# GeWu-Lab/Crab

Hardware: AMD Instinct MI355X
Metric: clips/sec prefill+decode (AVQA 10s clip, 8 frames, 256 out tok) (higher is better)
Workload: dtype bf16

## Files before the change

crab_amd/csrc/attn.hip:

```cpp
#include "common.h"
#include "crab_internal.h"
#include "attn_decode_core.h"
#include <math.h>
#include <stdlib.h>

namespace {

struct AttnP {
    const bf16_t* q; const bf16_t* k; const bf16_t* vt; bf16_t* o;
    long q_bs, q_hs, q_ss, k_bs, k_hs, k_ss, vt_bs, vt_hs, vt_ds, o_bs, o_ss;
    const float* bias; const float* gate;
    const int* kv_start;
    const uint32_t* key_mask; long key_mask_ld;
    int B, H, Hk, Sq, Skv, causal;
    float scale;
};

constexpr int KT = 64;
constexpr int VT_LD = 68;

template <int HD>
__device__ __forceinline__ int k_swz(int row, int chunk) {
    return HD == 128 ? (chunk ^ (row & 15)) : (HD == 64 ? (chunk ^ ((row >> 1) & 7)) : (chunk ^ ((0x78 >> (((row >> 2) & 3) * 2)) & 3)));
}

template <int HD, bool CAUSAL, bool BIAS>
__global__ __launch_bounds__(256) void attn_fwd_kernel(AttnP p) {
    constexpr int CPR = HD / 8;
    constexpr int KS = HD / 32;
    constexpr int DT = HD / 16;
    __shared__ __attribute__((aligned(16))) bf16_t lk[KT * HD];
    __shared__ __attribute__((aligned(16))) bf16_t lv[HD * VT_LD];

    const int tid = threadIdx.x, lane = tid & 63, wave = tid >> 6;
    const int fr = lane & 15, fg = lane >> 4;
    const int nqb = (p.Sq + 63) >> 6;
    const int lid = xcd_remap(blockIdx.x, gridDim.x);
    const int b = lid / (nqb * p.H), h = (lid / nqb) % p.H;
    const int hk = h / (p.H / p.Hk);
    const int q0 = (lid % nqb) * 64;
    const int qrow = q0 + wave * 16 + fr;
    const int qload = qrow < p.Sq ? qrow : p.Sq - 1;
    const int koff = p.Skv - p.Sq;

    const bf16_t* qp = p.q + (long)b * p.q_bs + (long)h * p.q_hs + (long)qload * p.q_ss;
    const bf16_t* kp = p.k + (long)b * p.k_bs + (long)hk * p.k_hs;
    const bf16_t* vp = p.vt + (long)b * p.vt_bs + (long)hk * p.vt_hs;

    bf16x8_t qf[KS];
#pragma unroll
    for (int ks = 0; ks < KS; ++ks) qf[ks] = *reinterpret_cast<const bf16x8_t*>(qp + ks * 32 + fg * 8);

    f32x4_t oacc[DT];
#pragma unroll
    for (int i = 0; i < DT; ++i) oacc[i] = f32x4_t{0.f, 0.f, 0.f, 0.f};
    float m_run = -1e30f, l_run = 0.f;

    float gate = 1.f;
    const float* biasrow = nullptr;
    if (BIAS) {
        if (p.gate) gate = p.gate[((long)b * p.H + h) * p.Sq + qload];
        biasrow = p.bias + ((long)h * p.Sq + qload) * p.Skv;
    }

    int kv_end = p.Skv;
    if (CAUSAL) {
        int last = q0 + 63 + koff;
        if (last + 1 < kv_end) kv_end = last + 1;
    }
    const int ntiles = (kv_end + KT - 1) / KT;
    const int ks0 = p.kv_start ? p.kv_start[b] : 0;
    const int t0 = ks0 / KT;
    const uint32_t* km = p.key_mask ? p.key_mask + (long)b * p.key_mask_ld : nullptr;

    constexpr int NKV = (KT * CPR) / 256, NVV = (HD * 8) / 256;
    u32x4 kreg[NKV], vreg[NVV];
#define ATT_LOAD_TILE(T_)                                                                                      \
    {                                                                                                          \
        const int kvl_ = (T_) * KT;                                                                            \
        _Pragma("unroll") for (int i = 0; i < NKV; ++i) {                                                      \
            const int idx = tid + i * 256;                                                                     \
            const int row = idx / CPR, c = idx % CPR;                                                          \
            const int kr = min(kvl_ + row, p.Skv - 1);                                                         \
            kreg[i] = *reinterpret_cast<const u32x4*>(kp + (long)kr * p.k_ss + c * 8);                         \
        }                                                                                                      \
        _Pragma("unroll") for (int i = 0; i < NVV; ++i) {                                                      \
            const int idx = tid + i * 256;                                                                     \
            const int row = idx >> 3, c = idx & 7;                                                             \
            int kc = kvl_ + c * 8;                          \
            kc = kc < p.Skv ? kc : 0;                                                                          \
            vreg[i] = *reinterpret_cast<const u32x4*>(vp + (long)row * p.vt_ds + kc);                          \
        }                                                                                                      \
    }
#define ATT_MASK_V(T_)                                                                                         \
    if ((T_) * KT + KT > p.Skv) {                                                                              \
        _Pragma("unroll") for (int i = 0; i < NVV; ++i) {                                                      \
            const int c = (tid + i * 256) & 7;                                                                 \
            const int rem = p.Skv - ((T_) * KT + c * 8);         \
            _Pragma("unroll") for (int w = 0; w < 4; ++w) {                                                    \
                const uint32_t m = (2 * w < rem ? 0x0000ffffu : 0u) | (2 * w + 1 < rem ? 0xffff0000u : 0u);    \
                vreg[i][w] &= m;                                                                               \
            }                                                                                                  \
        }                                                                                                      \
    }
    if (t0 < ntiles) ATT_LOAD_TILE(t0)
    for (int t = t0; t < ntiles; ++t) {
        const int kv0 = t * KT;
        __syncthreads();
        ATT_MASK_V(t)
#pragma unroll
        for (int i = 0; i < NKV; ++i) {
            const int idx = tid + i * 256;
            const int row = idx / CPR, c = idx % CPR;
            *reinterpret_cast<u32x4*>(lk + row * HD + (k_swz<HD>(row, c) << 3)) = kreg[i];
        }
#pragma unroll
        for (int i = 0; i < NVV; ++i) {
            const int idx = tid + i * 256;
            const int row = idx >> 3, c = idx & 7;
            bf16_t* d = lv + row * VT_LD + c * 8;
            *reinterpret_cast<u32x2*>(d) = u32x2{vreg[i][0], vreg[i][1]};
            *reinterpret_cast<u32x2*>(d + 4) = u32x2{vreg[i][2], vreg[i][3]};
        }
        __syncthreads();
        if (t + 1 < ntiles) ATT_LOAD_TILE(t + 1);

        f32x4_t s[4];
#pragma unroll
        for (int j = 0; j < 4; ++j) {
            s[j] = f32x4_t{0.f, 0.f, 0.f, 0.f};
#pragma unroll
            for (int ks = 0; ks < KS; ++ks) {
                int row = j * 16 + fr;
                int chunk = ks * 4 + fg;
                bf16x8_t kf = *reinterpret_cast<const bf16x8_t*>(lk + row * HD + (k_swz<HD>(row, chunk) << 3));
                s[j] = __builtin_amdgcn_mfma_f32_16x16x32_bf16(kf, qf[ks], s[j], 0, 0, 0);
            }
        }
        const float sc2 = p.scale * 1.4426950408889634f;
        const bool need_mask = (kv0 + KT > p.Skv) || (CAUSAL && (kv0 + KT - 1 > q0 + wave * 16 + koff)) || (kv0 < ks0) || km;
        float tmax = -1e30f;
        if (BIAS || need_mask) {
#pragma unroll
            for (int j = 0; j < 4; ++j) {
#pragma unroll
                for (int r = 0; r < 4; ++r) {
                    int kv = kv0 + j * 16 + fg * 4 + r;
                    float v = s[j][r] * sc2;
                    if (BIAS) { if (kv < p.Skv) v += gate * biasrow[kv] * 1.4426950408889634f; }
                    bool ok = kv < p.Skv && kv >= ks0;
// ... 14 lines not shown
        tmax = fmaxf(tmax, __shfl_xor(tmax, 16, 64));
        tmax = fmaxf(tmax, __shfl_xor(tmax, 32, 64));
        const float m_new = fmaxf(m_run, tmax);
        const float alpha = __builtin_amdgcn_exp2f(m_run - m_new);
        m_run = m_new;
        float psum = 0.f;
#pragma unroll
        for (int j = 0; j < 4; ++j)
#pragma unroll
            for (int r = 0; r < 4; ++r) {
                float e = __builtin_amdgcn_exp2f(s[j][r] - m_new);
                s[j][r] = e;
                psum += e;
            }
        l_run = l_run * alpha + psum;
#pragma unroll
        for (int i = 0; i < DT; ++i) oacc[i] *= alpha;

#pragma unroll
        for (int kk = 0; kk < 2; ++kk) {
            union { bf16x8_t v; uint32_t w[4]; } pf;
            pf.w[0] = pack_bf2(s[2 * kk][0], s[2 * kk][1]);
            pf.w[1] = pack_bf2(s[2 * kk][2], s[2 * kk][3]);
            pf.w[2] = pack_bf2(s[2 * kk + 1][0], s[2 * kk + 1][1]);
            pf.w[3] = pack_bf2(s[2 * kk + 1][2], s[2 * kk + 1][3]);
#pragma unroll
            for (int dt = 0; dt < DT; ++dt) {
                const bf16_t* vr = lv + (dt * 16 + fr) * VT_LD + kk * 32 + fg * 4;
                union { bf16x8_t v; u32x2 h[2]; } vf;
                vf.h[0] = *reinterpret_cast<const u32x2*>(vr);
                vf.h[1] = *reinterpret_cast<const u32x2*>(vr + 16);
                oacc[dt] = __builtin_amdgcn_mfma_f32_16x16x32_bf16(vf.v, pf.v, oacc[dt], 0, 0, 0);
            }
        }
    }
    l_run += __shfl_xor(l_run, 16, 64);
    l_run += __shfl_xor(l_run, 32, 64);
    const float inv = l_run > 0.f ? 1.0f / l_run : 0.f;
    if (qrow < p.Sq) {
        bf16_t* op = p.o + (long)b * p.o_bs + (long)qrow * p.o_ss + (long)h * HD;
#pragma unroll
        for (int dt = 0; dt < DT; ++dt) {
            u32x2 w;
            w[0] = pack_bf2(oacc[dt][0] * inv, oacc[dt][1] * inv);
            w[1] = pack_bf2(oacc[dt][2] * inv, oacc[dt][3] * inv);
            *reinterpret_cast<u32x2*>(op + dt * 16 + fg * 4) = w;
        }
    }
}


typedef __attribute__((ext_vector_type(16))) float f32x16_t;

template <int HD, bool CAUSAL>
__global__ __launch_bounds__(256, 2) void attn_fwd32_kernel(AttnP p) {
    constexpr int CPR = HD / 8;
    constexpr int KS = HD / 16;
    constexpr int DT = HD / 32;
    constexpr int KBUF = KT * HD, VBUF = HD * VT_LD;
    __shared__ __attribute__((aligned(16))) bf16_t lk[2 * KBUF];
    __shared__ __attribute__((aligned(16))) bf16_t lv[2 * VBUF];

    const int tid = threadIdx.x, lane = tid & 63;
    const int wave = __builtin_amdgcn_readfirstlane(tid >> 6);
    const int fc = lane & 31, fg = lane >> 5;
    const int nqb = (p.Sq + 127) >> 7;
    const int lid = xcd_remap(blockIdx.x, gridDim.x);
    const int b = lid / (nqb * p.H), h = (lid / nqb) % p.H;
    const int hk = h / (p.H / p.Hk);
    const int q0 = (nqb - 1 - lid % nqb) * 128;
    const int qw0 = q0 + wave * 32;
    const int qrow = qw0 + fc;
    const int qload = qrow < p.Sq ? qrow : p.Sq - 1;
    const int koff = p.Skv - p.Sq;
    const bool wave_on = qw0 < p.Sq;

    const bf16_t* qp = p.q + (long)b * p.q_bs + (long)h * p.q_hs + (long)qload * p.q_ss;
    const bf16_t* kp = p.k + (long)b * p.k_bs + (long)hk * p.k_hs;
    const bf16_t* vp = p.vt + (long)b * p.vt_bs + (long)hk * p.vt_hs;

    bf16x8_t qf[KS];
#pragma unroll
    for (int ks = 0; ks < KS; ++ks) qf[ks] = *reinterpret_cast<const bf16x8_t*>(qp + ks * 16 + fg * 8);

    f32x16_t oacc[DT];
#pragma unroll
    for (int i = 0; i < DT; ++i)
#pragma unroll
        for (int r = 0; r < 16; ++r) oacc[i][r] = 0.f;
    float m_run = -1e30f, l_run = 0.f;

    int kv_end = p.Skv;
    if (CAUSAL) kv_end = min(kv_end, q0 + 128 + koff);
    const int ntiles = (kv_end + KT - 1) / KT;
    const int ks0 = p.kv_start ? p.kv_start[b] : 0;
    const int t0 = ks0 / KT;
    const uint32_t* km = p.key_mask ? p.key_mask + (long)b * p.key_mask_ld : nullptr;
    constexpr int NKV = (KT * CPR) / 256, NVV = (HD * 8) / 256;
    u32x4 kreg[NKV], vreg[NVV];
#define ATT_STORE_TILE(BUF_, T_)                                                                               \
    {                                                                                                          \
        ATT_MASK_V(T_)                                                                                         \
        bf16_t* lk_ = lk + (BUF_) * KBUF;                                                                      \
        bf16_t* lv_ = lv + (BUF_) * VBUF;                                                                      \
        _Pragma("unroll") for (int i = 0; i < NKV; ++i) {                                                      \
            const int idx = tid + i * 256;                                                                     \
            const int row = idx / CPR, c = idx % CPR;                                                          \
            *reinterpret_cast<u32x4*>(lk_ + row * HD + (k_swz<HD>(row, c) << 3)) = kreg[i];                    \
        }                                                                                                      \
        _Pragma("unroll") for (int i = 0; i < NVV; ++i) {                                                      \
            const int idx = tid + i * 256;                                                                     \
            const int row = idx >> 3, c = idx & 7;                                                             \
            bf16_t* d_ = lv_ + row * VT_LD + c * 8;                                                            \
            *reinterpret_cast<u32x2*>(d_) = u32x2{vreg[i][0], vreg[i][1]};                                     \
            *reinterpret_cast<u32x2*>(d_ + 4) = u32x2{vreg[i][2], vreg[i][3]};                                 \
        }                                                                                                      \
    }
    if (t0 >= ntiles) {
        if (qrow < p.Sq) {
            bf16_t* op = p.o + (long)b * p.o_bs + (long)qrow * p.o_ss + (long)h * HD;
#pragma unroll
            for (int c = 0; c < HD / 4; ++c) *reinterpret_cast<u32x2*>(op + c * 4 + 0) = u32x2{0u, 0u};
        }
        return;
    }
    ATT_LOAD_TILE(t0)
    ATT_STORE_TILE(0, t0)
    if (t0 + 1 < ntiles) ATT_LOAD_TILE(t0 + 1)
    __syncthreads();
    const float sc2 = p.scale * 1.4426950408889634f;
    for (int t = t0; t < ntiles; ++t) {
        const int cur = (t - t0) & 1;
        const int kv0 = t * KT;
        if (t + 1 < ntiles) {
            ATT_STORE_TILE(cur ^ 1, t + 1)
            if (t + 2 < ntiles) ATT_LOAD_TILE(t + 2)
        }
        const bool skip = !wave_on || (CAUSAL && kv0 > qw0 + 31 + koff);
        if (!skip) {
            const bf16_t* lkc = lk + cur * KBUF;
            const bf16_t* lvc = lv + cur * VBUF;
            f32x16_t s[2];
#pragma unroll
            for (int j = 0; j < 2; ++j)
#pragma unroll
                for (int r = 0; r < 16; ++r) s[j][r] = 0.f;
#pragma unroll
            for (int ks = 0; ks < KS; ++ks) {
#pragma unroll
                for (int j = 0; j < 2; ++j) {
                    const int row = j * 32 + fc;
                    const int chunk = ks * 2 + fg;
                    bf16x8_t kf = *reinterpret_cast<const bf16x8_t*>(lkc + row * HD + (k_swz<HD>(row, chunk) << 3));
                    s[j] = __builtin_amdgcn_mfma_f32_32x32x16_bf16(kf, qf[ks], s[j], 0, 0, 0);
                }
            }
            const bool need_mask = (kv0 + KT > p.Skv) || (CAUSAL && (kv0 + KT - 1 > qw0 + koff)) || (kv0 < ks0) || km;
            if (need_mask) {
#pragma unroll
                for (int j = 0; j < 2; ++j)
#pragma unroll
                    for (int r = 0; r < 16; ++r) {
                        const int kv = kv0 + j * 32 + (r >> 2) * 8 + fg * 4 + (r & 3);
                        bool ok = kv < p.Skv && kv >= ks0;
                        if (CAUSAL) ok = ok && (kv <= qrow + koff);
                        if (km) ok = ok && ((km[min(kv, p.Skv - 1) >> 5] >> (kv & 31)) & 1u);
                        s[j][r] = ok ? s[j][r] : -INFINITY;
                    }
            }
            float tmax = -INFINITY;
#pragma unroll
            for (int j = 0; j < 2; ++j)
#pragma unroll
                for (int r = 0; r < 16; r += 2) tmax = fmaxf(tmax, fmaxf(s[j][r], s[j][r + 1]));
            tmax = fmaxf(tmax, __shfl_xor(tmax, 32, 64));
            const float m_new = fmaxf(m_run, tmax * sc2);
            const float alpha = __builtin_amdgcn_exp2f(m_run - m_new);
            const bool raised = m_new != m_run;
            m_run = m_new;
            float psum = 0.f;
#pragma unroll
            for (int j = 0; j < 2; ++j)
#pragma unroll
                for (int r = 0; r < 16; ++r) {
                    const float e = __builtin_amdgcn_exp2f(__builtin_fmaf(s[j][r], sc2, -m_new));
                    s[j][r] = e;
                    psum += e;
                }
            l_run = l_run * alpha + psum;
            if (__any(raised)) {
#pragma unroll
                for (int i = 0; i < DT; ++i) oacc[i] *= alpha;
            }
#pragma unroll
            for (int j = 0; j < 2; ++j)
#pragma unroll
                for (int kk = 0; kk < 2; ++kk) {
                    union { bf16x8_t v; uint32_t w[4]; } pf;
                    pf.w[0] = pack_bf2(s[j][8 * kk + 0], s[j][8 * kk + 1]);
                    pf.w[1] = pack_bf2(s[j][8 * kk + 2], s[j][8 * kk + 3]);
                    pf.w[2] = pack_bf2(s[j][8 * kk + 4], s[j][8 * kk + 5]);
                    pf.w[3] = pack_bf2(s[j][8 * kk + 6], s[j][8 * kk + 7]);
#pragma unroll
                    for (int dt = 0; dt < DT; ++dt) {
                        const bf16_t* vr = lvc + (dt * 32 + fc) * VT_LD + j * 32 + kk * 16 + fg * 4;
                        union { bf16x8_t v; u32x2 hh[2]; } vf;
                        vf.hh[0] = *reinterpret_cast<const u32x2*>(vr);
                        vf.hh[1] = *reinterpret_cast<const u32x2*>(vr + 8);
                        oacc[dt] = __builtin_amdgcn_mfma_f32_32x32x16_bf16(vf.v, pf.v, oacc[dt], 0, 0, 0);
                    }
                }
        }
        __syncthreads();
    }
    l_run += __shfl_xor(l_run, 32, 64);
    const float inv = l_run > 0.f ? 1.0f / l_run : 0.f;
    if (qrow < p.Sq) {
        bf16_t* op = p.o + (long)b * p.o_bs + (long)qrow * p.o_ss + (long)h * HD;
#pragma unroll
        for (int dt = 0; dt < DT; ++dt)
#pragma unroll
            for (int g4 = 0; g4 < 4; ++g4) {
                u32x2 w;
                w[0] = pack_bf2(oacc[dt][4 * g4 + 0] * inv, oacc[dt][4 * g4 + 1] * inv);
                w[1] = pack_bf2(oacc[dt][4 * g4 + 2] * inv, oacc[dt][4 * g4 + 3] * inv);
                *reinterpret_cast<u32x2*>(op + dt * 32 + g4 * 8 + fg * 4) = w;
            }
    }
}
#undef ATT_LOAD_TILE
#undef ATT_MASK_V
#undef ATT_STORE_TILE

template <int HD>
__global__ __launch_bounds__(256) void attn_decode_kernel(const bf16_t* __restrict__ q, long ldq, const bf16_t* __restrict__ kc,
                                                          const bf16_t* __restrict__ vc, bf16_t* __restrict__ o, long ldo, int H, int Hk,
                                                          int Tmax, int ctx_host, const int* __restrict__ ctx_dev, float scale,
                                                          const int* __restrict__ kv_start) {
    constexpr int EPL = HD / 16;
    const int tid = threadIdx.x;
    const int grp = tid >> 4, sub = tid & 15;
    const int b = blockIdx.y, h = blockIdx.x;
    const int hk = h / (H / Hk);
    const int ks0 = kv_start ? kv_start[b] : 0;
    const int ctx = ctx_host + (ctx_dev ? ctx_dev[0] : 0) - ks0;
    const bf16_t* qp = q + (long)b * ldq + (long)h * HD + sub * EPL;
    float qv[EPL];
#pragma unroll
    for (int e = 0; e < EPL; ++e) qv[e] = bf2f(qp[e]) * scale;
    const bf16_t* kb = kc + (((long)b * Hk + hk) * (long)Tmax + ks0) * HD + sub * EPL;
    const bf16_t* vb = vc + (((long)b * Hk + hk) * (long)Tmax + ks0) * HD + sub * EPL;
    float m = -1e30f, l = 0.f, acc[EPL];
#pragma unroll
    for (int e = 0; e < EPL; ++e) acc[e] = 0.f;
    if constexpr (EPL == 8) {
        dec_stream(qv, kb, vb, ctx, grp, m, l, acc);
    } else {
        for (int j = grp; j < ctx; j += 16) {
            float kx[EPL], vx[EPL];
            const u32x2 kw = __builtin_nontemporal_load(reinterpret_cast<const u32x2*>(kb + (long)j * HD));
            const u32x2 vw = __builtin_nontemporal_load(reinterpret_cast<const u32x2*>(vb + (long)j * HD));
#pragma unroll
            for (int e = 0; e < 2; ++e) { kx[2 * e] = lo_bf(kw[e]); kx[2 * e + 1] = hi_bf(kw[e]); vx[2 * e] = lo_bf(vw[e]); vx[2 * e + 1] = hi_bf(vw[e]); }
            float sdot = 0.f;
#pragma unroll
            for (int e = 0; e < EPL; ++e) sdot += qv[e] * kx[e];
            sdot = row16_sum(sdot);
            const float mn = fmaxf(m, sdot);
            const float a = __expf(m - mn), pw = __expf(sdot - mn);
            l = l * a + pw;
#pragma unroll
            for (int e = 0; e < EPL; ++e) acc[e] = acc[e] * a + pw * vx[e];
            m = mn;
        }
    }
    float M, L, O;
    dec_group_merge<HD, 16, EPL>(grp, sub, m, l, acc, M, L, O);
    if (tid < HD) o[(long)b * ldo + (long)h * HD + tid] = f2bf(O / L);
}


template <int HD>
__global__ __launch_bounds__(256) void attn_decode_keymask_kernel(const bf16_t* __restrict__ q, long ldq, const bf16_t* __restrict__ kc,
                                                                  const bf16_t* __restrict__ vc, bf16_t* __restrict__ o, long ldo, int H, int Hk,
                                                                  int Tmax, int ctx_host, const int* __restrict__ ctx_dev, float scale,
// ... 344 lines not shown
        }
        for (int r0 = 0; r0 < rounds; r0 += RPT) {
            if (r0 > 0) {
#pragma unroll
                for (int u = 0; u < RPT; ++u) {
                    const int jc = min((r0 + u) * 16 + grp, cn - 1);
                    vw[u] = __builtin_nontemporal_load(reinterpret_cast<const u32x4*>(vb + (long)(c0 + jc) * HD));
                }
            }
#pragma unroll
            for (int u = 0; u < RPT; ++u) {
                const int j = (r0 + u) * 16 + grp, jc = min(j, cn - 1);
                f32x4_t p0 = *reinterpret_cast<const f32x4_t*>(sbuf + jc * 8);
                f32x4_t p1 = *reinterpret_cast<const f32x4_t*>(sbuf + jc * 8 + 4);
                if (j >= cn) { p0 = f32x4_t{0.f, 0.f, 0.f, 0.f}; p1 = f32x4_t{0.f, 0.f, 0.f, 0.f}; }
                float vx[EPL];
#pragma unroll
                for (int e = 0; e < 4; ++e) { vx[2 * e] = lo_bf(vw[u][e]); vx[2 * e + 1] = hi_bf(vw[u][e]); }
#pragma unroll
                for (int g = 0; g < G; ++g) {
                    const float pg = g < 4 ? p0[g & 3] : p1[g & 3];
#pragma unroll
                    for (int e = 0; e < EPL; ++e) acc[g][e] += pg * vx[e];
                }
            }
        }
    }
    __syncthreads();
#pragma unroll
    for (int g = 0; g < G; ++g)
#pragma unroll
        for (int e = 0; e < EPL; ++e) {
            float v = acc[g][e];
            v += __shfl_xor(v, 16, 64);
            v += __shfl_xor(v, 32, 64);
            acc[g][e] = v;
        }
    if (lane < 16) {
#pragma unroll
        for (int g = 0; g < G; ++g)
#pragma unroll
            for (int e = 0; e < EPL; ++e) sbuf[(wave * G + g) * HD + sub * EPL + e] = acc[g][e];
    }
    __syncthreads();
    for (int idx = tid; idx < G * HD; idx += 256) {
        const float O = (sbuf[idx] + sbuf[G * HD + idx]) + (sbuf[2 * G * HD + idx] + sbuf[3 * G * HD + idx]);
        const int g = idx / HD;
        o[(long)b * ldo + (long)(hk * G) * HD + idx] = f2bf(O / l_run[g]);
    }
}

}

extern "C" int crab_attn_fwd(crab_ctx* ctx, void* stream, const crab_attn_desc* d) {
    if (!ctx) return CRAB_E_INVALID;
    if (!d || !d->q || !d->k || !d->vt || !d->o) return crab_fail(ctx, CRAB_E_INVALID, "attn_fwd: null operand");
    if (d->B <= 0 || d->H <= 0 || d->Hk <= 0 || d->H % d->Hk || d->Sq <= 0 || d->Skv <= 0)
        return crab_fail(ctx, CRAB_E_INVALID, "attn_fwd: bad shape");
    if (d->head_dim != 32 && d->head_dim != 64 && d->head_dim != 128) return crab_fail(ctx, CRAB_E_UNSUPPORTED, "attn_fwd: head_dim must be 32, 64 or 128");
    if (d->head_dim == 32 && (d->causal || d->bias)) return crab_fail(ctx, CRAB_E_UNSUPPORTED, "attn_fwd: head_dim 32 only without mask/bias");
    if ((d->q_ss & 7) || (d->q_hs & 7) || (d->q_bs & 7) || (d->k_ss & 7) || (d->k_hs & 7) || (d->k_bs & 7) || (d->vt_ds & 7) ||
        (d->vt_hs & 7) || (d->vt_bs & 7) || (d->o_ss & 3) || (d->o_bs & 3))
        return crab_fail(ctx, CRAB_E_INVALID, "attn_fwd: strides must keep 16-byte alignment");
    if (((uintptr_t)d->q & 15) || ((uintptr_t)d->k & 15) || ((uintptr_t)d->vt & 15) || ((uintptr_t)d->o & 7))
        return crab_fail(ctx, CRAB_E_INVALID, "attn_fwd: pointer alignment");
    if (d->causal && d->Skv < d->Sq) return crab_fail(ctx, CRAB_E_INVALID, "attn_fwd: causal needs Skv >= Sq");
    if ((d->bias == nullptr) && d->gate) return crab_fail(ctx, CRAB_E_INVALID, "attn_fwd: gate without bias");
    if (d->key_mask && (d->key_mask_ld < (d->Skv + 31) / 32 || d->head_dim == 32))
        return crab_fail(ctx, CRAB_E_INVALID, "attn_fwd: key_mask needs key_mask_ld >= ceil(Skv / 32) words per sequence (head_dim 64 / 128)");
    AttnP p;
    p.q = (const bf16_t*)d->q; p.k = (const bf16_t*)d->k; p.vt = (const bf16_t*)d->vt; p.o = (bf16_t*)d->o;
    p.q_bs = d->q_bs; p.q_hs = d->q_hs; p.q_ss = d->q_ss; p.k_bs = d->k_bs; p.k_hs = d->k_hs; p.k_ss = d->k_ss;
    p.vt_bs = d->vt_bs; p.vt_hs = d->vt_hs; p.vt_ds = d->vt_ds; p.o_bs = d->o_bs; p.o_ss = d->o_ss;
    p.bias = d->bias; p.gate = d->gate; p.kv_start = d->kv_start; p.key_mask = d->key_mask; p.key_mask_ld = d->key_mask_ld; p.B = d->B; p.H = d->H; p.Hk = d->Hk; p.Sq = d->Sq; p.Skv = d->Skv;
    p.causal = d->causal; p.scale = d->scale;
    dim3 grid(((d->Sq + 63) / 64) * d->H * d->B), block(256);
    hipStream_t s = (hipStream_t)stream;
    const bool hb = d->bias != nullptr;
    if (d->causal && hb) return crab_fail(ctx, CRAB_E_UNSUPPORTED, "attn_fwd: causal + bias not instantiated");
    static const int fwd32 = []() { const char* e = getenv("CRAB_ATTN_FWD32"); return !(e && e[0] == '0'); }();
    if (fwd32 && !hb && d->Sq > 64 && d->scale > 0.f && (d->head_dim == 128 || d->head_dim == 64)) {
        dim3 grid32(((d->Sq + 127) / 128) * d->H * d->B);
        if (d->head_dim == 128) {
            if (d->causal) hipLaunchKernelGGL((attn_fwd32_kernel<128, true>), grid32, block, 0, s, p);
            else hipLaunchKernelGGL((attn_fwd32_kernel<128, false>), grid32, block, 0, s, p);
        } else {
            if (d->causal) hipLaunchKernelGGL((attn_fwd32_kernel<64, true>), grid32, block, 0, s, p);
            else hipLaunchKernelGGL((attn_fwd32_kernel<64, false>), grid32, block, 0, s, p);
        }
        return crab_check_launch(ctx, d->head_dim == 128 ? (d->causal ? "attn_fwd32_kernel<128,causal>" : "attn_fwd32_kernel<128>")
                                                         : (d->causal ? "attn_fwd32_kernel<64,causal>" : "attn_fwd32_kernel<64>"));
    }
    if (d->head_dim == 32) {
        hipLaunchKernelGGL((attn_fwd_kernel<32, false, false>), grid, block, 0, s, p);
    } else if (d->head_dim == 128) {
        if (d->causal) hipLaunchKernelGGL((attn_fwd_kernel<128, true, false>), grid, block, 0, s, p);
        else if (hb) hipLaunchKernelGGL((attn_fwd_kernel<128, false, true>), grid, block, 0, s, p);
        else hipLaunchKernelGGL((attn_fwd_kernel<128, false, false>), grid, block, 0, s, p);
    } else {
        if (d->causal) hipLaunchKernelGGL((attn_fwd_kernel<64, true, false>), grid, block, 0, s, p);
        else if (hb) hipLaunchKernelGGL((attn_fwd_kernel<64, false, true>), grid, block, 0, s, p);
        else hipLaunchKernelGGL((attn_fwd_kernel<64, false, false>), grid, block, 0, s, p);
    }
    return crab_check_launch(ctx, d->head_dim == 32 ? "attn_fwd_kernel<32>" : d->head_dim == 128 ? (d->causal ? "attn_fwd_kernel<128,causal>" : hb ? "attn_fwd_kernel<128,bias>" : "attn_fwd_kernel<128>")
                                                                            : (d->causal ? "attn_fwd_kernel<64,causal>" : hb ? "attn_fwd_kernel<64,bias>" : "attn_fwd_kernel<64>"));
}

extern "C" int64_t crab_attn_decode_rope_workspace(int B, int H, int d) {
    return ((int64_t)B * H * 8 * (d + 2) * 4 + 255) / 256 * 256 + (int64_t)B * H * 4;
}

extern "C" int crab_attn_decode_rope(crab_ctx* ctx, void* stream, const void* qkv, int64_t ldqkv, const float* rope_tab, void* k_cache,
                                     void* v_cache, void* o, int64_t ldo, int B, int H, int Hk, int d, int Tmax, int pos0,
                                     const int32_t* pos_dev, float scale, void* workspace, int64_t workspace_bytes) {
    if (!ctx) return CRAB_E_INVALID;
    if (!qkv || !rope_tab || !k_cache || !v_cache || !o || B <= 0 || H <= 0 || Hk <= 0 || H % Hk) return crab_fail(ctx, CRAB_E_INVALID, "attn_decode_rope: bad argument");
    if (d != 64 && d != 128) return crab_fail(ctx, CRAB_E_UNSUPPORTED, "attn_decode_rope: head_dim must be 64 or 128");
    if ((ldqkv & 7) || ((uintptr_t)qkv & 15) || ((uintptr_t)k_cache & 15) || ((uintptr_t)v_cache & 15)) return crab_fail(ctx, CRAB_E_INVALID, "attn_decode_rope: alignment");
    if (!pos_dev && (pos0 < 0 || pos0 >= Tmax)) return crab_fail(ctx, CRAB_E_INVALID, "attn_decode_rope: position outside the KV cache");
    int nsplit = 1;
    static const int tgt = []() { const char* e = getenv("CRAB_ATTN_BLOCKS"); return e ? atoi(e) : 512; }();
    if ((long)B * H < tgt) { nsplit = (int)(tgt / ((long)B * H)); if (nsplit > 8) nsplit = 8; }
    if (nsplit > 1 && (!workspace || workspace_bytes < crab_attn_decode_rope_workspace(B, H, d)))
        return crab_fail(ctx, CRAB_E_WORKSPACE, "attn_decode_rope: needs crab_attn_decode_rope_workspace(B, H, d) bytes (counters zeroed once)");
    float* part = (float*)workspace;
    unsigned* counters = workspace ? (unsigned*)((char*)workspace + ((int64_t)B * H * 8 * (d + 2) * 4 + 255) / 256 * 256) : nullptr;
    hipStream_t s = (hipStream_t)stream;
    static const int wide_on = []() { const char* e = getenv("CRAB_ATTN_WIDE"); return !(e && e[0] == '0'); }();
    if (wide_on && nsplit == 2 && d == 128) {
        hipLaunchKernelGGL((attn_decode_rope_kernel<128, 32>), dim3(H, B, 1), dim3(512), 0, s, (const bf16_t*)qkv, (long)ldqkv, rope_tab, (bf16_t*)k_cache,
                           (bf16_t*)v_cache, (bf16_t*)o, (long)ldo, H, Hk, Tmax, pos0, pos_dev, scale, (float*)nullptr, (unsigned*)nullptr);
        return crab_check_launch(ctx, "attn_decode_rope_kernel<128,32>");
    }
    dim3 grid(H, B, nsplit), block(256);
    if (d == 128)
        hipLaunchKernelGGL((attn_decode_rope_kernel<128>), grid, block, 0, s, (const bf16_t*)qkv, (long)ldqkv, rope_tab, (bf16_t*)k_cache,
                           (bf16_t*)v_cache, (bf16_t*)o, (long)ldo, H, Hk, Tmax, pos0, pos_dev, scale, part, counters);
    else
        hipLaunchKernelGGL((attn_decode_rope_kernel<64>), grid, block, 0, s, (const bf16_t*)qkv, (long)ldqkv, rope_tab, (bf16_t*)k_cache,
                           (bf16_t*)v_cache, (bf16_t*)o, (long)ldo, H, Hk, Tmax, pos0, pos_dev, scale, part, counters);
    return crab_check_launch(ctx, d == 128 ? "attn_decode_rope_kernel<128>" : "attn_decode_rope_kernel<64>");
}

extern "C" int crab_attn_decode_keymask(crab_ctx* ctx, void* stream, const void* q, int64_t ldq, const void* k_cache, const void* v_cache,
                                        void* o, int64_t ldo, int B, int H, int Hk, int d, int Tmax, int ctx_len_host, const int32_t* ctx_dev,
                                        float scale, const uint32_t* key_mask, int64_t key_mask_ld) {
    if (!ctx) return CRAB_E_INVALID;
    if (!q || !k_cache || !v_cache || !o || !key_mask || B <= 0 || H <= 0 || Hk <= 0 || H % Hk) return crab_fail(ctx, CRAB_E_INVALID, "attn_decode_keymask: bad argument");
    if (d != 64 && d != 128) return crab_fail(ctx, CRAB_E_UNSUPPORTED, "attn_decode_keymask: head_dim must be 64 or 128");
    if (!ctx_dev && (ctx_len_host <= 0 || ctx_len_host > Tmax)) return crab_fail(ctx, CRAB_E_INVALID, "attn_decode_keymask: ctx_len out of range");
    if (key_mask_ld < ((ctx_dev ? Tmax : ctx_len_host) + 31) / 32)
        return crab_fail(ctx, CRAB_E_INVALID, "attn_decode_keymask: key_mask_ld must cover the visible context (ceil(ctx_len / 32) words, Tmax with ctx_dev)");
    dim3 grid(H, B), block(256);
    hipStream_t s = (hipStream_t)stream;
    if (d == 128)
        hipLaunchKernelGGL((attn_decode_keymask_kernel<128>), grid, block, 0, s, (const bf16_t*)q, (long)ldq, (const bf16_t*)k_cache, (const bf16_t*)v_cache,
                           (bf16_t*)o, (long)ldo, H, Hk, Tmax, ctx_len_host, ctx_dev, scale, key_mask, (long)key_mask_ld);
    else
        hipLaunchKernelGGL((attn_decode_keymask_kernel<64>), grid, block, 0, s, (const bf16_t*)q, (long)ldq, (const bf16_t*)k_cache, (const bf16_t*)v_cache,
// ... 38 lines not shown
```

crab_amd/csrc/crab_internal.h:

```cpp
#pragma once
#include <hip/hip_runtime.h>
#include <stdio.h>
#include <string.h>
#include "../../include/crab_hip.h"

#define CRAB_TRACE_MAX 160
struct crab_trace_row { char name[64]; long count; };
struct crab_ctx {
    int device;
    char err[512];
    int trace_on;
    int trace_n;
    crab_trace_row trace[CRAB_TRACE_MAX];
};

static inline void crab_trace_note(crab_ctx* ctx, const char* what) {
    for (int i = 0; i < ctx->trace_n; ++i)
        if (strncmp(ctx->trace[i].name, what, sizeof(ctx->trace[i].name) - 1) == 0) { ++ctx->trace[i].count; return; }
    if (ctx->trace_n >= CRAB_TRACE_MAX) return;
    crab_trace_row* r = &ctx->trace[ctx->trace_n++];
    strncpy(r->name, what, sizeof(r->name) - 1);
    r->name[sizeof(r->name) - 1] = 0;
    r->count = 1;
}

static inline int crab_fail(crab_ctx* ctx, int code, const char* msg) {
    if (ctx) { strncpy(ctx->err, msg, sizeof(ctx->err) - 1); ctx->err[sizeof(ctx->err) - 1] = 0; }
    return code;
}

static inline int crab_check_launch(crab_ctx* ctx, const char* what) {
    hipError_t e = hipGetLastError();
    if (e != hipSuccess) {
        if (ctx) snprintf(ctx->err, sizeof(ctx->err), "%s: %s", what, hipGetErrorString(e));
        return CRAB_E_HIP;
    }
    if (ctx && ctx->trace_on) crab_trace_note(ctx, what);
    return CRAB_OK;
}

#define CRAB_HIP_TRY(ctx, expr)                                                                  \
    do {                                                                                         \
        hipError_t _e = (expr);                                                                  \
        if (_e != hipSuccess) {                                                                  \
            if (ctx) snprintf((ctx)->err, sizeof((ctx)->err), "%s: %s", #expr, hipGetErrorString(_e)); \
            return CRAB_E_HIP;                                                                   \
        }                                                                                        \
    } while (0)

static inline int crab_cflags(const crab_gemm_desc* d) { return (d->c_fp32 ? 1 : 0) | ((d->r_fp32 && d->R) ? 2 : 0); }

bool crab_rowfin_enabled();
extern "C" int crab_rowfin_lora_ok(int nl, int r, int N);
```

crab_amd/csrc/encoder_layers.hip:

```cpp
#include "crab_internal.h"
#include <math.h>

namespace {

int dense(crab_ctx* ctx, void* stream, const crab_enc_io* io, const crab_dense* w, const void* a, int64_t lda, void* c, int64_t ldc, int M, int act,
          const void* residual, int64_t ldr, float res_scale, int c_fp32 = 0, int r_fp32 = 0) {
    crab_gemm_desc d;
    memset(&d, 0, sizeof(d));
    d.A = a; d.lda = lda; d.B = w->W; d.ldb = w->ldw; d.C = c; d.ldc = ldc; d.bias = w->bias;
    d.R = residual; d.ldr = ldr; d.res_scale = res_scale; d.c_fp32 = c_fp32; d.r_fp32 = residual ? r_fp32 : 0;
    d.M = M; d.N = w->N; d.K = w->K; d.act = act; d.batch = 1; d.nb0 = 1;
    if (M <= CRAB_DECODE_MAX_ROWS) { d.workspace = io->workspace; d.workspace_bytes = io->workspace_bytes; }
    return crab_gemm_bf16(ctx, stream, &d);
}

int attention(crab_ctx* ctx, void* stream, const crab_enc_io* io, const uint16_t* q, int64_t ldq, const uint16_t* k, int64_t ldk,
              void* vsrc, int64_t ldv, int v_skip, int B, int H, int Sq, int Skv, int d, const float* bias, const float* gate) {
    const int Sp = (Skv + 7) / 8 * 8;
    if ((int64_t)B * H * d * Sp * 2 > io->vt_bytes) return crab_fail(ctx, CRAB_E_WORKSPACE, "encoder layer: vt scratch smaller than B * H * d * round8(Skv) * 2 bytes");
    int rc = crab_qkv_rope_split(ctx, stream, vsrc, ldv, nullptr, nullptr, nullptr, io->vt, Sp, B, Skv, v_skip, H, d, 1, 0, nullptr);
    if (rc) return rc;
    crab_attn_desc a;
    memset(&a, 0, sizeof(a));
    a.q = q; a.k = k; a.vt = io->vt; a.o = io->att;
    a.q_bs = (int64_t)Sq * ldq; a.q_hs = d; a.q_ss = ldq;
    a.k_bs = (int64_t)Skv * ldk; a.k_hs = d; a.k_ss = ldk;
    a.vt_bs = (int64_t)H * d * Sp; a.vt_hs = (int64_t)d * Sp; a.vt_ds = Sp;
    a.o_bs = (int64_t)Sq * H * d; a.o_ss = (int64_t)H * d;
    a.bias = bias; a.gate = gate;
    a.B = B; a.H = H; a.Hk = H; a.Sq = Sq; a.Skv = Skv; a.head_dim = d; a.causal = 0;
    a.scale = (float)(1.0 / sqrt((double)d));
    return crab_attn_fwd(ctx, stream, &a);
}

int ln(crab_ctx* ctx, void* stream, int x_fp32, const void* x, int64_t ldx, const crab_ln* w, void* y, int64_t ldy, int M, int D) {
    return crab_layernorm_p(ctx, stream, x, x_fp32, ldx, w->w, w->b, w->fp32, y, ldy, M, D, w->eps);
}

int check_io(crab_ctx* ctx, const crab_enc_io* io, bool need_f, const char* who) {
    char msg[160];
    if (!io || !io->x || !io->a || !io->qkv || !io->att || !io->vt || !io->y || (need_f && !io->f) || io->B <= 0 || io->S <= 0) {
        snprintf(msg, sizeof(msg), "%s: x, a, qkv, att, vt, y%s and positive B, S are required", who, need_f ? ", f" : "");
        return crab_fail(ctx, CRAB_E_INVALID, msg);
    }
    return CRAB_OK;
}

}

extern "C" {

int crab_clip_layer(crab_ctx* ctx, void* stream, const crab_clip_layer_w* w, crab_enc_io* io) {
    if (!ctx) return CRAB_E_INVALID;
    if (!w) return crab_fail(ctx, CRAB_E_INVALID, "clip_layer: null weights");
    int rc = check_io(ctx, io, true, "clip_layer");
    if (rc) return rc;
    const int D = w->out.N, H = w->H, M = io->B * io->S;
    if (H <= 0 || D % H || w->qkv.N != 3 * D || w->qkv.K != D || w->out.K != D || w->fc1.K != D || w->fc2.N != D || w->fc2.K != w->fc1.N)
        return crab_fail(ctx, CRAB_E_INVALID, "clip_layer: shapes do not chain (qkv [3D, D], out [D, D], fc1 [I, D], fc2 [D, I])");
    const int d = D / H;
    uint16_t* qkv = (uint16_t*)io->qkv;
    const int xf = io->x_fp32 ? 1 : 0;
    if ((rc = ln(ctx, stream, xf, io->x, D, &w->ln1, io->a, D, M, D))) return rc;
    if ((rc = dense(ctx, stream, io, &w->qkv, io->a, D, qkv, 3 * D, M, CRAB_ACT_NONE, nullptr, 0, 1.0f))) return rc;
    if ((rc = attention(ctx, stream, io, qkv, 3 * D, qkv + D, 3 * D, qkv, 3 * D, H, io->B, H, io->S, io->S, d, nullptr, nullptr))) return rc;
    if ((rc = dense(ctx, stream, io, &w->out, io->att, D, io->y, D, M, CRAB_ACT_NONE, io->x, D, 1.0f, xf, xf))) return rc;
    if ((rc = ln(ctx, stream, xf, io->y, D, &w->ln2, io->a, D, M, D))) return rc;
    if ((rc = dense(ctx, stream, io, &w->fc1, io->a, D, io->f, w->fc1.N, M, CRAB_ACT_QUICK_GELU, nullptr, 0, 1.0f))) return rc;
    return dense(ctx, stream, io, &w->fc2, io->f, w->fc1.N, io->x, D, M, CRAB_ACT_NONE, io->y, D, 1.0f, xf, xf);
}

int crab_beats_layer(crab_ctx* ctx, void* stream, const crab_beats_layer_w* w, crab_enc_io* io) {
    if (!ctx) return CRAB_E_INVALID;
    if (!w) return crab_fail(ctx, CRAB_E_INVALID, "beats_layer: null weights");
    int rc = check_io(ctx, io, true, "beats_layer");
    if (rc) return rc;
    const int E = w->out.N, H = w->H, M = io->B * io->S;
    if (H <= 0 || E % H || w->qkv.N != 3 * E || w->qkv.K != E || w->out.K != E || w->fc1.K != E || w->fc2.N != E || w->fc2.K != w->fc1.N)
        return crab_fail(ctx, CRAB_E_INVALID, "beats_layer: shapes do not chain (qkv [3E, E], out [E, E], fc1 [F, E], fc2 [E, F])");
    if (w->grep_w && (!w->grep_b || !w->grep_a || !io->gate || !io->bias)) return crab_fail(ctx, CRAB_E_INVALID, "beats_layer: the gated bias needs grep_b, grep_a, io->gate and io->bias");
    const int d = E / H;
    uint16_t* qkv = (uint16_t*)io->qkv;
    if ((rc = dense(ctx, stream, io, &w->qkv, io->x, E, qkv, 3 * E, M, CRAB_ACT_NONE, nullptr, 0, 1.0f))) return rc;
    const float* gate = nullptr;
// ... 48 lines not shown
```

Measured before the change: 30.88.

## Read row-major V in encoder attention and split short query tails into a one-wave kernel

```diff
diff --git a/crab_amd/csrc/attn.hip b/crab_amd/csrc/attn.hip
--- a/crab_amd/csrc/attn.hip
+++ b/crab_amd/csrc/attn.hip
@@ -14,6 +14,7 @@
     const uint32_t* key_mask; long key_mask_ld;
     int B, H, Hk, Sq, Skv, causal;
     float scale;
+    int nqb;
 };
 
 constexpr int KT = 64;
@@ -73,19 +74,20 @@
     const int t0 = ks0 / KT;
     const uint32_t* km = p.key_mask ? p.key_mask + (long)b * p.key_mask_ld : nullptr;
 
-    constexpr int NKV = (KT * CPR) / 256, NVV = (HD * 8) / 256;
+    constexpr int NT = 256;
+    constexpr int NKV = (KT * CPR) / NT, NVV = (HD * 8) / NT;
     u32x4 kreg[NKV], vreg[NVV];
 #define ATT_LOAD_TILE(T_)                                                                                      \
     {                                                                                                          \
         const int kvl_ = (T_) * KT;                                                                            \
         _Pragma("unroll") for (int i = 0; i < NKV; ++i) {                                                      \
-            const int idx = tid + i * 256;                                                                     \
+            const int idx = tid + i * NT;                                                                      \
             const int row = idx / CPR, c = idx % CPR;                                                          \
             const int kr = min(kvl_ + row, p.Skv - 1);                                                         \
             kreg[i] = *reinterpret_cast<const u32x4*>(kp + (long)kr * p.k_ss + c * 8);                         \
         }                                                                                                      \
         _Pragma("unroll") for (int i = 0; i < NVV; ++i) {                                                      \
-            const int idx = tid + i * 256;                                                                     \
+            const int idx = tid + i * NT;                                                                      \
             const int row = idx >> 3, c = idx & 7;                                                             \
             int kc = kvl_ + c * 8;                          \
             kc = kc < p.Skv ? kc : 0;                                                                          \
@@ -95,7 +97,7 @@
 #define ATT_MASK_V(T_)                                                                                         \
     if ((T_) * KT + KT > p.Skv) {                                                                              \
         _Pragma("unroll") for (int i = 0; i < NVV; ++i) {                                                      \
-            const int c = (tid + i * 256) & 7;                                                                 \
+            const int c = (tid + i * NT) & 7;                                                                  \
             const int rem = p.Skv - ((T_) * KT + c * 8);         \
             _Pragma("unroll") for (int w = 0; w < 4; ++w) {                                                    \
                 const uint32_t m = (2 * w < rem ? 0x0000ffffu : 0u) | (2 * w + 1 < rem ? 0xffff0000u : 0u);    \
@@ -216,8 +218,8 @@
 
 typedef __attribute__((ext_vector_type(16))) float f32x16_t;
 
-template <int HD, bool CAUSAL>
-__global__ __launch_bounds__(256, 2) void attn_fwd32_kernel(AttnP p) {
+template <int HD, bool CAUSAL, int NW = 4, bool VROW = false>
+__global__ __launch_bounds__(NW * 64, NW == 4 ? 2 : 1) void attn_fwd32_kernel(AttnP p) {
     constexpr int CPR = HD / 8;
     constexpr int KS = HD / 16;
     constexpr int DT = HD / 32;
@@ -228,11 +230,12 @@
     const int tid = threadIdx.x, lane = tid & 63;
     const int wave = __builtin_amdgcn_readfirstlane(tid >> 6);
     const int fc = lane & 31, fg = lane >> 5;
-    const int nqb = (p.Sq + 127) >> 7;
+    const int nqb = NW == 4 ? p.nqb : 1;
     const int lid = xcd_remap(blockIdx.x, gridDim.x);
     const int b = lid / (nqb * p.H), h = (lid / nqb) % p.H;
     const int hk = h / (p.H / p.Hk);
-    const int q0 = (nqb - 1 - lid % nqb) * 128;
+    const int q0 = NW == 4 ? (nqb - 1 - lid % nqb) * 128
+                           : (p.Sq >> 7) * 128;
     const int qw0 = q0 + wave * 32;
     const int qrow = qw0 + fc;
     const int qload = qrow < p.Sq ? qrow : p.Sq - 1;
@@ -260,20 +263,65 @@
     const int ks0 = p.kv_start ? p.kv_start[b] : 0;
     const int t0 = ks0 / KT;
     const uint32_t* km = p.key_mask ? p.key_mask + (long)b * p.key_mask_ld : nullptr;
-    constexpr int NKV = (KT * CPR) / 256, NVV = (HD * 8) / 256;
+    constexpr int NT = NW * 64;
+    constexpr int NKV = (KT * CPR) / NT, NVV = (HD * 8) / NT;
     u32x4 kreg[NKV], vreg[NVV];
+#define ATT_LOAD_TILE_VR(T_)                                                                                   \
+    {                                                                                                          \
+        const int kvl_ = (T_) * KT;                                                                            \
+        _Pragma("unroll") for (int i = 0; i < NKV; ++i) {                                                      \
+            const int idx = tid + i * NT;                                                                      \
+            const int row = idx / CPR, c = idx % CPR;                                                          \
+            const int kr = min(kvl_ + row, p.Skv - 1);                                                         \
+            kreg[i] = *reinterpret_cast<const u32x4*>(kp + (long)kr * p.k_ss + c * 8);                         \
+        }                                                                                                      \
+        _Pragma("unroll") for (int i = 0; i < NVV / 2; ++i) {                                                  \
+            const int idx = tid + i * NT;                                                                      \
+            const int kp_ = idx / CPR, c = idx % CPR;                                                          \
+            const int r0 = min(kvl_ + 2 * kp_, p.Skv - 1), r1 = min(kvl_ + 2 * kp_ + 1, p.Skv - 1);            \
+            vreg[2 * i] = *reinterpret_cast<const u32x4*>(vp + (long)r0 * p.vt_ds + c * 8);                    \
+            vreg[2 * i + 1] = *reinterpret_cast<const u32x4*>(vp + (long)r1 * p.vt_ds + c * 8);                \
+        }                                                                                                      \
+    }
+#define ATT_STORE_TILE_VR(BUF_, T_)                                                                            \
+    {                                                                                                          \
+        if ((T_) * KT + KT > p.Skv) {                                                                          \
+            _Pragma("unroll") for (int i = 0; i < NVV; ++i) {                                                  \
+                const int key = (T_) * KT + 2 * ((tid + (i >> 1) * NT) / CPR) + (i & 1);                       \
+                const uint32_t m = key < p.Skv ? 0xffffffffu : 0u;                                             \
+                _Pragma("unroll") for (int w = 0; w < 4; ++w) vreg[i][w] &= m;                                 \
+            }                                                                                                  \
+        }                                                                                                      \
+        bf16_t* lk_ = lk + (BUF_) * KBUF;                                                                      \
+        bf16_t* lv_ = lv + (BUF_) * VBUF;                                                                      \
+        _Pragma("unroll") for (int i = 0; i < NKV; ++i) {                                                      \
+            const int idx = tid + i * NT;                                                                      \
+            const int row = idx / CPR, c = idx % CPR;                                                          \
+            *reinterpret_cast<u32x4*>(lk_ + row * HD + (k_swz<HD>(row, c) << 3)) = kreg[i];                    \
+        }                                                                                                      \
+        _Pragma("unroll") for (int i = 0; i < NVV / 2; ++i) {                                                  \
+            const int idx = tid + i * NT;                                                                      \
+            const int kp_ = idx / CPR, c = idx % CPR;                                                          \
+            bf16_t* d_ = lv_ + (c * 8) * VT_LD + 2 * kp_;                                                      \
+            _Pragma("unroll") for (int w = 0; w < 4; ++w) {         \
+                const uint32_t a_ = vreg[2 * i][w], b_ = vreg[2 * i + 1][w];                                   \
+                *reinterpret_cast<uint32_t*>(d_ + (2 * w) * VT_LD) = __builtin_amdgcn_perm(b_, a_, 0x05040100u);      \
+                *reinterpret_cast<uint32_t*>(d_ + (2 * w + 1) * VT_LD) = __builtin_amdgcn_perm(b_, a_, 0x07060302u);  \
+            }                                                                                                  \
+        }                                                                                                      \
+    }
 #define ATT_STORE_TILE(BUF_, T_)                                                                               \
     {                                                                                                          \
         ATT_MASK_V(T_)                                                                                         \
         bf16_t* lk_ = lk + (BUF_) * KBUF;                                                                      \
         bf16_t* lv_ = lv + (BUF_) * VBUF;                                                                      \
         _Pragma("unroll") for (int i = 0; i < NKV; ++i) {                                                      \
-            const int idx = tid + i * 256;                                                                     \
+            const int idx = tid + i * NT;                                                                      \
             const int row = idx / CPR, c = idx % CPR;                                                          \
             *reinterpret_cast<u32x4*>(lk_ + row * HD + (k_swz<HD>(row, c) << 3)) = kreg[i];                    \
         }                                                                                                      \
         _Pragma("unroll") for (int i = 0; i < NVV; ++i) {                                                      \
-            const int idx = tid + i * 256;                                                                     \
+            const int idx = tid + i * NT;                                                                      \
             const int row = idx >> 3, c = idx & 7;                                                             \
             bf16_t* d_ = lv_ + row * VT_LD + c * 8;                                                            \
             *reinterpret_cast<u32x2*>(d_) = u32x2{vreg[i][0], vreg[i][1]};                                     \
@@ -288,17 +336,19 @@
         }
         return;
     }
-    ATT_LOAD_TILE(t0)
-    ATT_STORE_TILE(0, t0)
-    if (t0 + 1 < ntiles) ATT_LOAD_TILE(t0 + 1)
+#define ATT32_LOAD(T_) { if constexpr (VROW) ATT_LOAD_TILE_VR(T_) else ATT_LOAD_TILE(T_) }
+#define ATT32_STORE(BUF_, T_) { if constexpr (VROW) ATT_STORE_TILE_VR(BUF_, T_) else ATT_STORE_TILE(BUF_, T_) }
+    ATT32_LOAD(t0)
+    ATT32_STORE(0, t0)
+    if (t0 + 1 < ntiles) ATT32_LOAD(t0 + 1)
     __syncthreads();
     const float sc2 = p.scale * 1.4426950408889634f;
     for (int t = t0; t < ntiles; ++t) {
         const int cur = (t - t0) & 1;
         const int kv0 = t * KT;
         if (t + 1 < ntiles) {
-            ATT_STORE_TILE(cur ^ 1, t + 1)
-            if (t + 2 < ntiles) ATT_LOAD_TILE(t + 2)
+            ATT32_STORE(cur ^ 1, t + 1)
+            if (t + 2 < ntiles) ATT32_LOAD(t + 2)
         }
         const bool skip = !wave_on || (CAUSAL && kv0 > qw0 + 31 + koff);
         if (!skip) {
@@ -395,6 +445,10 @@
 #undef ATT_LOAD_TILE
 #undef ATT_MASK_V
 #undef ATT_STORE_TILE
+#undef ATT_LOAD_TILE_VR
+#undef ATT_STORE_TILE_VR
+#undef ATT32_LOAD
+#undef ATT32_STORE
 
 template <int HD>
 __global__ __launch_bounds__(256) void attn_decode_kernel(const bf16_t* __restrict__ q, long ldq, const bf16_t* __restrict__ kc,
@@ -845,7 +899,16 @@
 
 }
 
-extern "C" int crab_attn_fwd(crab_ctx* ctx, void* stream, const crab_attn_desc* d) {
+static bool attn_fwd32_on() {
+    static const int on = []() { const char* e = getenv("CRAB_ATTN_FWD32"); return !(e && e[0] == '0'); }();
+    return on;
+}
+
+bool crab_attn_fwd_vrows_ok(int Sq, int head_dim, bool has_bias) {
+    return attn_fwd32_on() && !has_bias && Sq > 64 && (head_dim == 64 || head_dim == 128);
+}
+
+static int attn_fwd_impl(crab_ctx* ctx, void* stream, const crab_attn_desc* d, bool vrows) {
     if (!ctx) return CRAB_E_INVALID;
     if (!d || !d->q || !d->k || !d->vt || !d->o) return crab_fail(ctx, CRAB_E_INVALID, "attn_fwd: null operand");
     if (d->B <= 0 || d->H <= 0 || d->Hk <= 0 || d->H % d->Hk || d->Sq <= 0 || d->Skv <= 0)
@@ -866,23 +929,44 @@
     p.q_bs = d->q_bs; p.q_hs = d->q_hs; p.q_ss = d->q_ss; p.k_bs = d->k_bs; p.k_hs = d->k_hs; p.k_ss = d->k_ss;
     p.vt_bs = d->vt_bs; p.vt_hs = d->vt_hs; p.vt_ds = d->vt_ds; p.o_bs = d->o_bs; p.o_ss = d->o_ss;
     p.bias = d->bias; p.gate = d->gate; p.kv_start = d->kv_start; p.key_mask = d->key_mask; p.key_mask_ld = d->key_mask_ld; p.B = d->B; p.H = d->H; p.Hk = d->Hk; p.Sq = d->Sq; p.Skv = d->Skv;
-    p.causal = d->causal; p.scale = d->scale;
+    p.causal = d->causal; p.scale = d->scale; p.nqb = 0;
     dim3 grid(((d->Sq + 63) / 64) * d->H * d->B), block(256);
     hipStream_t s = (hipStream_t)stream;
     const bool hb = d->bias != nullptr;
     if (d->causal && hb) return crab_fail(ctx, CRAB_E_UNSUPPORTED, "attn_fwd: causal + bias not instantiated");
-    static const int fwd32 = []() { const char* e = getenv("CRAB_ATTN_FWD32"); return !(e && e[0] == '0'); }();
+    const bool fwd32 = attn_fwd32_on();
+    if (vrows && !(crab_attn_fwd_vrows_ok(d->Sq, d->head_dim, hb) && d->scale > 0.f && !d->causal))
+        return crab_fail(ctx, CRAB_E_UNSUPPORTED, "attn_fwd: row-major V only on the 128-row kernel (no bias, not causal, Sq > 64, head_dim 64 / 128)");
     if (fwd32 && !hb && d->Sq > 64 && d->scale > 0.f && (d->head_dim == 128 || d->head_dim == 64)) {
-        dim3 grid32(((d->Sq + 127) / 128) * d->H * d->B);
+        static const int tail_on = []() { const char* e = getenv("CRAB_ATTN_TAIL"); return !(e && e[0] == '0'); }();
+        const int rem = d->Sq & 127;
+        const bool tail = tail_on && d->Sq > 128 && rem >= 1 && rem <= 32;
+        p.nqb = tail ? d->Sq >> 7 : (d->Sq + 127) >> 7;
+        dim3 grid32(p.nqb * d->H * d->B);
         if (d->head_dim == 128) {
             if (d->causal) hipLaunchKernelGGL((attn_fwd32_kernel<128, true>), grid32, block, 0, s, p);
+            else if (vrows) hipLaunchKernelGGL((attn_fwd32_kernel<128, false, 4, true>), grid32, block, 0, s, p);
             else hipLaunchKernelGGL((attn_fwd32_kernel<128, false>), grid32, block, 0, s, p);
         } else {
             if (d->causal) hipLaunchKernelGGL((attn_fwd32_kernel<64, true>), grid32, block, 0, s, p);
+            else if (vrows) hipLaunchKernelGGL((attn_fwd32_kernel<64, false, 4, true>), grid32, block, 0, s, p);
             else hipLaunchKernelGGL((attn_fwd32_kernel<64, false>), grid32, block, 0, s, p);
         }
-        return crab_check_launch(ctx, d->head_dim == 128 ? (d->causal ? "attn_fwd32_kernel<128,causal>" : "attn_fwd32_kernel<128>")
-                                                         : (d->causal ? "attn_fwd32_kernel<64,causal>" : "attn_fwd32_kernel<64>"));
+        int rc = crab_check_launch(ctx, d->head_dim == 128 ? (d->causal ? "attn_fwd32_kernel<128,causal>" : "attn_fwd32_kernel<128>")
+                                                           : (d->causal ? "attn_fwd32_kernel<64,causal>" : "attn_fwd32_kernel<64>"));
+        if (rc || !tail) return rc;
+        dim3 gridt(d->H * d->B), blockt(64);
+        if (d->head_dim == 128) {
+            if (d->causal) hipLaunchKernelGGL((attn_fwd32_kernel<128, true, 1>), gridt, blockt, 0, s, p);
+            else if (vrows) hipLaunchKernelGGL((attn_fwd32_kernel<128, false, 1, true>), gridt, blockt, 0, s, p);
+            else hipLaunchKernelGGL((attn_fwd32_kernel<128, false, 1>), gridt, blockt, 0, s, p);
+        } else {
+            if (d->causal) hipLaunchKernelGGL((attn_fwd32_kernel<64, true, 1>), gridt, blockt, 0, s, p);
+            else if (vrows) hipLaunchKernelGGL((attn_fwd32_kernel<64, false, 1, true>), gridt, blockt, 0, s, p);
+            else hipLaunchKernelGGL((attn_fwd32_kernel<64, false, 1>), gridt, blockt, 0, s, p);
+        }
+        return crab_check_launch(ctx, d->head_dim == 128 ? (d->causal ? "attn_fwd32_tail_kernel<128,causal>" : "attn_fwd32_tail_kernel<128>")
+                                                         : (d->causal ? "attn_fwd32_tail_kernel<64,causal>" : "attn_fwd32_tail_kernel<64>"));
     }
     if (d->head_dim == 32) {
         hipLaunchKernelGGL((attn_fwd_kernel<32, false, false>), grid, block, 0, s, p);
@@ -898,6 +982,10 @@
     return crab_check_launch(ctx, d->head_dim == 32 ? "attn_fwd_kernel<32>" : d->head_dim == 128 ? (d->causal ? "attn_fwd_kernel<128,causal>" : hb ? "attn_fwd_kernel<128,bias>" : "attn_fwd_kernel<128>")
                                                                             : (d->causal ? "attn_fwd_kernel<64,causal>" : hb ? "attn_fwd_kernel<64,bias>" : "attn_fwd_kernel<64>"));
 }
+
+extern "C" int crab_attn_fwd(crab_ctx* ctx, void* stream, const crab_attn_desc* d) { return attn_fwd_impl(ctx, stream, d, false); }
+
+int crab_attn_fwd_vrows(crab_ctx* ctx, void* stream, const crab_attn_desc* d) { return attn_fwd_impl(ctx, stream, d, true); }
 
 extern "C" int64_t crab_attn_decode_rope_workspace(int B, int H, int d) {
     return ((int64_t)B * H * 8 * (d + 2) * 4 + 255) / 256 * 256 + (int64_t)B * H * 4;
diff --git a/crab_amd/csrc/crab_internal.h b/crab_amd/csrc/crab_internal.h
--- a/crab_amd/csrc/crab_internal.h
+++ b/crab_amd/csrc/crab_internal.h
@@ -50,5 +50,9 @@
 
 static inline int crab_cflags(const crab_gemm_desc* d) { return (d->c_fp32 ? 1 : 0) | ((d->r_fp32 && d->R) ? 2 : 0); }
 
+#define CRAB_HIDDEN __attribute__((visibility("hidden")))
+CRAB_HIDDEN bool crab_attn_fwd_vrows_ok(int Sq, int head_dim, bool has_bias);
+CRAB_HIDDEN int crab_attn_fwd_vrows(crab_ctx* ctx, void* stream, const crab_attn_desc* d);
+
 bool crab_rowfin_enabled();
 extern "C" int crab_rowfin_lora_ok(int nl, int r, int N);
diff --git a/crab_amd/csrc/encoder_layers.hip b/crab_amd/csrc/encoder_layers.hip
--- a/crab_amd/csrc/encoder_layers.hip
+++ b/crab_amd/csrc/encoder_layers.hip
@@ -16,20 +16,26 @@
 
 int attention(crab_ctx* ctx, void* stream, const crab_enc_io* io, const uint16_t* q, int64_t ldq, const uint16_t* k, int64_t ldk,
               void* vsrc, int64_t ldv, int v_skip, int B, int H, int Sq, int Skv, int d, const float* bias, const float* gate) {
+    crab_attn_desc a;
+    memset(&a, 0, sizeof(a));
+    a.q = q; a.o = io->att; a.k = k;
+    a.q_bs = (int64_t)Sq * ldq; a.q_hs = d; a.q_ss = ldq;
+    a.k_bs = (int64_t)Skv * ldk; a.k_hs = d; a.k_ss = ldk;
+    a.o_bs = (int64_t)Sq * H * d; a.o_ss = (int64_t)H * d;
+    a.bias = bias; a.gate = gate;
+    a.B = B; a.H = H; a.Hk = H; a.Sq = Sq; a.Skv = Skv; a.head_dim = d; a.causal = 0;
+    a.scale = (float)(1.0 / sqrt((double)d));
+    if (crab_attn_fwd_vrows_ok(Sq, d, bias != nullptr) && !(ldv & 7)) {
+        a.vt = (const uint16_t*)vsrc + (int64_t)(v_skip + H) * d;
+        a.vt_bs = (int64_t)Skv * ldv; a.vt_hs = d; a.vt_ds = ldv;
+        return crab_attn_fwd_vrows(ctx, stream, &a);
+    }
     const int Sp = (Skv + 7) / 8 * 8;
     if ((int64_t)B * H * d * Sp * 2 > io->vt_bytes) return crab_fail(ctx, CRAB_E_WORKSPACE, "encoder layer: vt scratch smaller than B * H * d * round8(Skv) * 2 bytes");
     int rc = crab_qkv_rope_split(ctx, stream, vsrc, ldv, nullptr, nullptr, nullptr, io->vt, Sp, B, Skv, v_skip, H, d, 1, 0, nullptr);
     if (rc) return rc;
-    crab_attn_desc a;
-    memset(&a, 0, sizeof(a));
-    a.q = q; a.k = k; a.vt = io->vt; a.o = io->att;
-    a.q_bs = (int64_t)Sq * ldq; a.q_hs = d; a.q_ss = ldq;
-    a.k_bs = (int64_t)Skv * ldk; a.k_hs = d; a.k_ss = ldk;
+    a.vt = io->vt;
     a.vt_bs = (int64_t)H * d * Sp; a.vt_hs = (int64_t)d * Sp; a.vt_ds = Sp;
-    a.o_bs = (int64_t)Sq * H * d; a.o_ss = (int64_t)H * d;
-    a.bias = bias; a.gate = gate;
-    a.B = B; a.H = H; a.Hk = H; a.Sq = Sq; a.Skv = Skv; a.head_dim = d; a.causal = 0;
-    a.scale = (float)(1.0 / sqrt((double)d));
     return crab_attn_fwd(ctx, stream, &a);
 }
 
```

Result: no change. 31.02 (median of 6 runs) (+0.5%).
